# rezashkv/unlearn-ft

Measured on AMD Instinct MI355X. Metric: bilevel train-step images/sec @512^2 pruned-SD2.1, higher is better.
Workload: dtype bf16; 1 GPU; BASELINE configs[1] model+batch (MAC-budget-0.55 SD-2.1 student [ratio 0.556, 223.7 GMAC/img] + dense teacher [402.1 GMAC/img], B=8/GPU, 64x64 latents = 512^2 px, losses 1.0 ddpm(min-SNR 5) + 2.0 distill + 0.1 block) under the bilevel cadence of configs[2] (upper concept-suppression step every 10th iteration, second AdamW); global_batch=8, parallelism=dp1, student_params=483766084, weights=random-init, attention_precision=activation dtype, dist_backend=none, rccl_ranks=0, dp_mode=allreduce, teacher_prefetch=True

## Files before the change

unlearn-ft_amd/csrc/attention.hip:

```cpp
#include <cstdlib>

#include "common.h"

namespace {

constexpr int NT = 256;
constexpr int D = 64;
constexpr float LOG2E = 1.4426950408889634f;
typedef __attribute__((ext_vector_type(4))) unsigned u32x4;
typedef __attribute__((ext_vector_type(2))) float f32x2;
constexpr unsigned OOB = 0x80000000u;

#ifndef PDMK_ATTN_KVB
#define PDMK_ATTN_KVB 64
#endif
template <typename T> struct ACfg;
template <> struct ACfg<bf16> {
    static constexpr int CH = 8, RS = 64, KVB = PDMK_ATTN_KVB;
};
template <> struct ACfg<float> {
    static constexpr int CH = 4, RS = 68, KVB = 32;
};

template <typename T> struct AT;
template <> struct AT<bf16> {
    typedef Mma<bf16> MM;
    static constexpr int RS = 64;
    static __device__ __forceinline__ int sw(int row) { return row & 7; }
    static __device__ __forceinline__ MM::frag rowk(const bf16* lds, int row0, int k0, int lane) {
        const int row = row0 + (lane & 15), ch = ((k0 >> 3) + (lane >> 4)) ^ (row & 7);
        return *reinterpret_cast<const bf16x8*>(lds + row * RS + ch * 8);
    }
    template <int S> static __device__ __forceinline__ MM::frag colk_accs(const bf16* lds, int k0, int col0, int lane) {
        const int g = lane >> 4, q = (lane & 15) >> 2, p = lane & 3;
        const int row = k0 + 4 * g + q;
        const bf16* a0 = lds + row * RS + ((((col0 >> 3) + (p >> 1)) ^ (row & 7)) * 8) + (p & 1) * 4;
        typedef __attribute__((address_space(3))) s16x4 lds_s16x4;
        s16x4 lo = __builtin_amdgcn_ds_read_tr16_b64_v4i16((lds_s16x4*)(a0));
        s16x4 hi = __builtin_amdgcn_ds_read_tr16_b64_v4i16((lds_s16x4*)(a0 + 16 * RS));
        s16x8 v = __builtin_shufflevector(lo, hi, 0, 1, 2, 3, 4, 5, 6, 7);
        return __builtin_bit_cast(bf16x8, v);
    }
};
template <> struct AT<float> {
    typedef Mma<float> MM;
    static constexpr int RS = 68;
    static __device__ __forceinline__ int sw(int) { return 0; }
    static __device__ __forceinline__ MM::frag rowk(const float* lds, int row0, int k0, int lane) {
        return MM::load_rowk(lds, RS, row0, k0, lane);
    }
    template <int S> static __device__ __forceinline__ MM::frag colk_accs(const float* lds, int k0, int col0, int lane) {
        return MM::template load_colk_accs<S>(lds, RS, k0, col0, lane);
    }
};

template <typename T, int ROWS> struct TileIO {
    static constexpr int CH = ACfg<T>::CH, RS = ACfg<T>::RS, CPR = D / CH, NR = ROWS * CPR / NT;
    static_assert(ROWS * CPR % NT == 0, "tile chunks must divide the block");
    template <typename RS_T>
    static __device__ __forceinline__ void load(u32x4* r, const RS_T& rsrc, int ld, int row0, int nrows, int tid) {
#pragma unroll
        for (int i = 0; i < NR; ++i) {
            const int c = tid + i * NT, row = row0 + c / CPR, dc = (c % CPR) * CH;
            const unsigned off = row < nrows ? ((unsigned)row * (unsigned)ld + (unsigned)dc) * (unsigned)sizeof(T) : OOB;
            r[i] = __builtin_amdgcn_raw_buffer_load_b128(rsrc, (int)off, 0, 0);
        }
    }
    static __device__ __forceinline__ void store(T* lds, const u32x4* r, int tid) {
#pragma unroll
        for (int i = 0; i < NR; ++i) {
            const int c = tid + i * NT, row = c / CPR;
            *reinterpret_cast<u32x4*>(lds + row * RS + (((c % CPR) ^ AT<T>::sw(row)) * CH)) = r[i];
        }
    }
};

template <typename T> __device__ __forceinline__ auto make_rsrc(const T* p, long nrows, int ld) {
    const long bytes = ((nrows - 1) * (long)ld + D) * (long)sizeof(T);
    return __builtin_amdgcn_make_buffer_rsrc(const_cast<T*>(p), (short)0, (int)bytes, 0x00020000);
}

template <typename T>
__device__ __forceinline__ void store_tile16(const T* lds, T* g, long ld, int row0, int nrows, int lane) {
    constexpr int CH = ACfg<T>::CH, RS = ACfg<T>::RS, CPR = D / CH;
    for (int c = lane; c < 16 * CPR; c += 64) {
        const int r = c / CPR, dc = (c % CPR) * CH;
        if (row0 + r < nrows)
            *reinterpret_cast<uint4*>(g + (long)(row0 + r) * ld + dc) = *reinterpret_cast<const uint4*>(lds + r * RS + dc);
    }
}
template <typename T>
__device__ __forceinline__ void stage_t(T* lds, const f32x4* acc, float scale, int lane) {
    constexpr int RS = ACfg<T>::RS;
#pragma unroll
    for (int dt = 0; dt < 4; ++dt)
#pragma unroll
        for (int r = 0; r < 4; ++r)
            lds[(lane & 15) * RS + dt * 16 + (lane >> 4) * 4 + r] = from_f32<T>(acc[dt][r] * scale);
}

template <typename MM, int S, int NS> struct AccLoop {
    template <typename F> static __device__ __forceinline__ void run(F&& f) {
        f(std::integral_constant<int, S>{});
        AccLoop<MM, S + 1, NS>::run(f);
    }
};
template <typename MM, int NS> struct AccLoop<MM, NS, NS> {
    template <typename F> static __device__ __forceinline__ void run(F&&) {}
};

template <typename T> struct BlockSums : std::is_same<T, float> {};

template <typename T, int NQ, bool CAUSAL = false>
__global__ __launch_bounds__(NT) void attn_fwd_kernel(const T* __restrict__ q, const T* __restrict__ k,
                                                      const T* __restrict__ v, T* __restrict__ o,
                                                      float* __restrict__ lse, int H, int Nq, int Nk, long q_bs,
                                                      int q_ld, long k_bs, int k_ld, long v_bs, int v_ld, long o_bs,
                                                      int o_ld, float scale2) {
    typedef Mma<T> MM;
    typedef ACfg<T> AC;
    constexpr int RS = AC::RS, KVB = AC::KVB, NKT = KVB / 16, QROWS = 64 * NQ;
    constexpr bool BLOCK_SUMS = BlockSums<T>::value;
    typedef TileIO<T, QROWS> QIO;
    typedef TileIO<T, KVB> KIO;
    __shared__ __attribute__((aligned(16))) T Qs[QROWS * RS];
    __shared__ __attribute__((aligned(16))) T Ks[2][KVB * RS];
    __shared__ __attribute__((aligned(16))) T Vs[2][KVB * RS];

    const int tid = threadIdx.x, lane = tid & 63, wave = tid >> 6;
    const int q0 = blockIdx.x * QROWS, h = blockIdx.y, b = blockIdx.z;
    const auto rq = make_rsrc(q + b * q_bs + h * D, Nq, q_ld);
    const auto rk = make_rsrc(k + b * k_bs + h * D, Nk, k_ld);
    const auto rv = make_rsrc(v + b * v_bs + h * D, Nk, v_ld);

    u32x4 rk_[KIO::NR], rv_[KIO::NR];
    {
        u32x4 rq_[QIO::NR];
        QIO::load(rq_, rq, q_ld, q0, Nq, tid);
        KIO::load(rk_, rk, k_ld, 0, Nk, tid);
        KIO::load(rv_, rv, v_ld, 0, Nk, tid);
        QIO::store(Qs, rq_, tid);
    }
    KIO::store(Ks[0], rk_, tid);
    KIO::store(Vs[0], rv_, tid);
    __syncthreads();
    typename MM::frag qf[NQ][D / MM::KS];
#pragma unroll
    for (int n = 0; n < NQ; ++n)
#pragma unroll
        for (int kk = 0; kk < D / MM::KS; ++kk) qf[n][kk] = AT<T>::rowk(Qs, (wave * NQ + n) * 16, kk * MM::KS, lane);

    f32x4 ot[NQ][4], ol[NQ];
    float m_run[NQ];
#pragma unroll
    for (int n = 0; n < NQ; ++n) {
        m_run[n] = -INFINITY;
        ol[n] = f32x4{0.f, 0.f, 0.f, 0.f};
#pragma unroll
        for (int i = 0; i < 4; ++i) ot[n][i] = f32x4{0.f, 0.f, 0.f, 0.f};
    }
    typename MM::frag ones;
    if constexpr (std::is_same<T, bf16>::value) {
#pragma unroll
        for (int e = 0; e < 8; ++e) ones[e] = (bf16)1.0f;
    } else {
        ones = 1.0f;
    }

    int cur = 0;
    auto block = [&](auto tail_c, const int kb) {
        constexpr bool TAIL = decltype(tail_c)::value;
        const bool more = kb + KVB < Nk;
        if (more) {
            KIO::load(rk_, rk, k_ld, kb + KVB, Nk, tid);
            KIO::load(rv_, rv, v_ld, kb + KVB, Nk, tid);
        }
        f32x4 st[NQ][NKT];
#pragma unroll
        for (int t = 0; t < NKT; ++t) {
#pragma unroll
            for (int n = 0; n < NQ; ++n) st[n][t] = f32x4{0.f, 0.f, 0.f, 0.f};
#pragma unroll
            for (int kk = 0; kk < D / MM::KS; ++kk) {
                const typename MM::frag kf = AT<T>::rowk(Ks[cur], t * 16, kk * MM::KS, lane);
#pragma unroll
                for (int n = 0; n < NQ; ++n) st[n][t] = MM::mma(kf, qf[n][kk], st[n][t]);
            }
        }
#pragma unroll
        for (int n = 0; n < NQ; ++n) {
            float mx = -INFINITY;
            if (TAIL) {
#pragma unroll
                for (int t = 0; t < NKT; ++t)
#pragma unroll
                    for (int r = 0; r < 4; ++r)
                        if (kb + t * 16 + (lane >> 4) * 4 + r >= Nk) st[n][t][r] = -INFINITY;
            }
            if (CAUSAL) {
                const int qi = q0 + (wave * NQ + n) * 16 + (lane & 15);
#pragma unroll
                for (int t = 0; t < NKT; ++t)
#pragma unroll
                    for (int r = 0; r < 4; ++r)
                        if (kb + t * 16 + (lane >> 4) * 4 + r > qi) st[n][t][r] = -INFINITY;
            }
#pragma unroll
            for (int t = 0; t < NKT; ++t)
#pragma unroll
                for (int r = 0; r < 4; ++r) mx = fmaxf(mx, st[n][t][r]);
            mx = fmaxf(mx, __shfl_xor(mx, 16, 64));
            mx = fmaxf(mx, __shfl_xor(mx, 32, 64));
            const float mxs = mx * scale2;
            const bool move = mxs > m_run[n] + 8.0f;
            if (__builtin_amdgcn_ballot_w64(move)) {
                const float mn = move ? mxs : m_run[n];
                const float alpha = __builtin_amdgcn_exp2f(m_run[n] - mn);
                m_run[n] = mn;
#pragma unroll
                for (int r = 0; r < 4; ++r) ol[n][r] *= alpha;
#pragma unroll
                for (int dt = 0; dt < 4; ++dt)
#pragma unroll
                    for (int r = 0; r < 4; ++r) ot[n][dt][r] *= alpha;
            }
            const f32x2 sc2 = {scale2, scale2}, nm2 = {-m_run[n], -m_run[n]};
#pragma unroll
            for (int t = 0; t < NKT; ++t)
#pragma unroll
                for (int r = 0; r < 4; r += 2) {
                    const f32x2 e2 = __builtin_elementwise_fma(f32x2{st[n][t][r], st[n][t][r + 1]}, sc2, nm2);
                    st[n][t][r] = __builtin_amdgcn_exp2f(e2[0]);
                    st[n][t][r + 1] = __builtin_amdgcn_exp2f(e2[1]);
                }
        }
        f32x4 otb[BLOCK_SUMS ? NQ : 1][4], olb[BLOCK_SUMS ? NQ : 1];
        if constexpr (BLOCK_SUMS) {
#pragma unroll
            for (int n = 0; n < NQ; ++n) {
                olb[n] = f32x4{0.f, 0.f, 0.f, 0.f};
#pragma unroll
                for (int i = 0; i < 4; ++i) otb[n][i] = f32x4{0.f, 0.f, 0.f, 0.f};
            }
        }
#pragma unroll
        for (int pr = 0; pr < NKT / 2; ++pr) {
            AccLoop<MM, 0, MM::ACC_STEPS>::run([&](auto sc) {
                constexpr int S = decltype(sc)::value;
                typename MM::frag pf[NQ];
#pragma unroll
                for (int n = 0; n < NQ; ++n) {
                    pf[n] = MM::template acc_frag<S>(st[n][2 * pr], st[n][2 * pr + 1]);
                    if constexpr (BLOCK_SUMS) olb[n] = MM::mma(ones, pf[n], olb[n]);
                    else ol[n] = MM::mma(ones, pf[n], ol[n]);
                }
#pragma unroll
                for (int dt = 0; dt < 4; ++dt) {
                    const typename MM::frag vf = AT<T>::template colk_accs<S>(Vs[cur], pr * 32, dt * 16, lane);
#pragma unroll
                    for (int n = 0; n < NQ; ++n) {
                        if constexpr (BLOCK_SUMS) otb[n][dt] = MM::mma(vf, pf[n], otb[n][dt]);
                        else ot[n][dt] = MM::mma(vf, pf[n], ot[n][dt]);
                    }
                }
            });
        }
        if constexpr (BLOCK_SUMS) {
#pragma unroll
            for (int n = 0; n < NQ; ++n) {
                ol[n] += olb[n];
#pragma unroll
                for (int dt = 0; dt < 4; ++dt) ot[n][dt] += otb[n][dt];
            }
        }
        if (more) {
            KIO::store(Ks[cur ^ 1], rk_, tid);
            KIO::store(Vs[cur ^ 1], rv_, tid);
        }
        __syncthreads();
        cur ^= 1;
    };
    const int nfull = Nk / KVB * KVB;
    for (int kb = 0; kb < nfull; kb += KVB) block(std::false_type{}, kb);
    if (nfull < Nk) block(std::true_type{}, nfull);
#pragma unroll
    for (int n = 0; n < NQ; ++n) {
        const float l = ol[n][0];
        T* Ow = Qs + (wave * NQ + n) * 16 * RS;
        stage_t<T>(Ow, ot[n], 1.0f / l, lane);
        const int qi = q0 + (wave * NQ + n) * 16 + (lane & 15);
        if (lane < 16 && qi < Nq) lse[((long)b * H + h) * Nq + qi] = m_run[n] + log2f(l);
    }
    __syncthreads();
#pragma unroll
    for (int n = 0; n < NQ; ++n)
        store_tile16<T>(Qs + (wave * NQ + n) * 16 * RS, o + b * o_bs + h * D, o_ld, q0 + (wave * NQ + n) * 16, Nq, lane);
}

template <typename T>
__global__ void attn_delta_kernel(const T* __restrict__ o, const T* __restrict__ d_o, float* __restrict__ delta, int H,
                                  int Nq, long o_bs, int o_ld, long total) {
    constexpr int CH = ACfg<T>::CH;
    for (long i = blockIdx.x * (long)NT + threadIdx.x; i < total; i += (long)gridDim.x * NT) {
        const int qi = (int)(i % Nq);
        const long bh = i / Nq;
        const int h = (int)(bh % H);
        const long b = bh / H;
        const T* po = o + b * o_bs + (long)qi * o_ld + h * D;
        const T* pd = d_o + b * o_bs + (long)qi * o_ld + h * D;
        float s = 0.f;
#pragma unroll
        for (int c = 0; c < D; c += CH) {
            const uint4 a = *reinterpret_cast<const uint4*>(po + c), g = *reinterpret_cast<const uint4*>(pd + c);
            const T* ae = reinterpret_cast<const T*>(&a);
            const T* ge = reinterpret_cast<const T*>(&g);
#pragma unroll
            for (int e = 0; e < CH; ++e) s += to_f32(ae[e]) * to_f32(ge[e]);
        }
        delta[i] = s;
    }
}

template <typename T, bool SPLIT, int NKW>
__global__ __launch_bounds__(NT) void attn_bwd_dkv_kernel(const T* __restrict__ q, const T* __restrict__ k,
                                                          const T* __restrict__ v, const T* __restrict__ d_o,
                                                          const float* __restrict__ lse,
                                                          const float* __restrict__ delta, T* __restrict__ dk,
                                                          T* __restrict__ dv, int H, int Nq, int Nk, long q_bs,
                                                          int q_ld, long k_bs, int k_ld, long v_bs, int v_ld,
                                                          long o_bs, int o_ld, long dk_bs, int dk_ld, long dv_bs,
                                                          int dv_ld, float scale, float scale2, float* __restrict__ ws,
                                                          int nsplit) {
    typedef Mma<T> MM;
    typedef ACfg<T> AC;
    constexpr int RS = AC::RS, QB = AC::KVB, NQT = QB / 16, KROWS = 64 * NKW;
    constexpr bool BLOCK_SUMS = BlockSums<T>::value;
    typedef TileIO<T, KROWS> KIO;
    typedef TileIO<T, QB> QIO;
    static_assert(!SPLIT || NKW == 1, "the query split is for few-key grids");
    __shared__ __attribute__((aligned(16))) T Ks[KROWS * RS];
    __shared__ __attribute__((aligned(16))) T Vs[KROWS * RS];
    __shared__ __attribute__((aligned(16))) T Qs[2][QB * RS];
    __shared__ __attribute__((aligned(16))) T Os[2][QB * RS];
    __shared__ __attribute__((aligned(16))) float Ls[2][QB], Ds[2][QB];

    const int tid = threadIdx.x, lane = tid & 63, wave = tid >> 6;
    const int kblocks = (Nk + KROWS - 1) / KROWS;
    const int split = SPLIT ? blockIdx.x / kblocks : 0;
    const int k0 = (SPLIT ? blockIdx.x - split * kblocks : blockIdx.x) * KROWS, h = blockIdx.y, b = blockIdx.z;
    int q_begin = 0, q_end = Nq;
    if (SPLIT) {
        const int nqb = (Nq + QB - 1) / QB, per = (nqb + nsplit - 1) / nsplit;
        q_begin = min(Nq, split * per * QB);
        q_end = min(Nq, (split + 1) * per * QB);
    }
    const auto rq = make_rsrc(q + b * q_bs + h * D, Nq, q_ld);
    const auto ro = make_rsrc(d_o + b * o_bs + h * D, Nq, o_ld);
    const auto rk = make_rsrc(k + b * k_bs + h * D, Nk, k_ld);
    const auto rv = make_rsrc(v + b * v_bs + h * D, Nk, v_ld);
    const float* lse_bh = lse + ((long)b * H + h) * Nq;
    const float* del_bh = delta + ((long)b * H + h) * Nq;

    u32x4 rq_[QIO::NR], ro_[QIO::NR];
    float rl = -INFINITY, rd = 0.f;
    {
        u32x4 rk_[KIO::NR], rv_[KIO::NR];
        KIO::load(rk_, rk, k_ld, k0, Nk, tid);
        KIO::load(rv_, rv, v_ld, k0, Nk, tid);
        QIO::load(rq_, rq, q_ld, q_begin, Nq, tid);
        QIO::load(ro_, ro, o_ld, q_begin, Nq, tid);
        if (tid < QB && q_begin + tid < Nq) { rl = -lse_bh[q_begin + tid]; rd = -del_bh[q_begin + tid]; }
        KIO::store(Ks, rk_, tid);
        KIO::store(Vs, rv_, tid);
    }
    QIO::store(Qs[0], rq_, tid);
    QIO::store(Os[0], ro_, tid);
    if (tid < QB) { Ls[0][tid] = rl; Ds[0][tid] = rd; }
    __syncthreads();
    typename MM::frag kf[NKW][D / MM::KS], vf[NKW][D / MM::KS];
    f32x4 dkt[NKW][4], dvt[NKW][4];
#pragma unroll
    for (int j = 0; j < NKW; ++j) {
#pragma unroll
        for (int kk = 0; kk < D / MM::KS; ++kk) {
            kf[j][kk] = AT<T>::rowk(Ks, (wave * NKW + j) * 16, kk * MM::KS, lane);
            vf[j][kk] = AT<T>::rowk(Vs, (wave * NKW + j) * 16, kk * MM::KS, lane);
        }
#pragma unroll
        for (int i = 0; i < 4; ++i) { dkt[j][i] = f32x4{0.f, 0.f, 0.f, 0.f}; dvt[j][i] = f32x4{0.f, 0.f, 0.f, 0.f}; }
    }

    int cur = 0;
    for (int qb = q_begin; qb < q_end; qb += QB) {
        const bool more = qb + QB < q_end;
        if (more) {
            QIO::load(rq_, rq, q_ld, qb + QB, Nq, tid);
            QIO::load(ro_, ro, o_ld, qb + QB, Nq, tid);
            rl = -INFINITY; rd = 0.f;
            if (tid < QB && qb + QB + tid < Nq) { rl = -lse_bh[qb + QB + tid]; rd = -del_bh[qb + QB + tid]; }
        }
        f32x4 p[NKW][NQT], ds[NKW][NQT];
#pragma unroll
        for (int t = 0; t < NQT; ++t) {
            f32x4 sacc[NKW], dp[NKW];
            const f32x4 nd = *reinterpret_cast<const f32x4*>(&Ds[cur][t * 16 + (lane >> 4) * 4]);
            const f32x4 nlv = *reinterpret_cast<const f32x4*>(&Ls[cur][t * 16 + (lane >> 4) * 4]);
#pragma unroll
            for (int j = 0; j < NKW; ++j) { sacc[j] = f32x4{0.f, 0.f, 0.f, 0.f}; dp[j] = BLOCK_SUMS ? f32x4{0.f, 0.f, 0.f, 0.f} : nd; }
#pragma unroll
            for (int kk = 0; kk < D / MM::KS; ++kk) {
                const typename MM::frag qa = AT<T>::rowk(Qs[cur], t * 16, kk * MM::KS, lane);
                const typename MM::frag oa = AT<T>::rowk(Os[cur], t * 16, kk * MM::KS, lane);
#pragma unroll
                for (int j = 0; j < NKW; ++j) {
                    sacc[j] = MM::mma(qa, kf[j][kk], sacc[j]);
                    dp[j] = MM::mma(oa, vf[j][kk], dp[j]);
                }
            }
#pragma unroll
            for (int r = 0; r < 4; r += 2) {
#pragma unroll
                for (int j = 0; j < NKW; ++j) {
                    const f32x2 e2 = __builtin_elementwise_fma(f32x2{sacc[j][r], sacc[j][r + 1]}, f32x2{scale2, scale2}, f32x2{nlv[r], nlv[r + 1]});
                    const f32x2 pv = {__builtin_amdgcn_exp2f(e2[0]), __builtin_amdgcn_exp2f(e2[1])};
                    f32x2 dpd = {dp[j][r], dp[j][r + 1]};
                    if constexpr (BLOCK_SUMS) dpd += f32x2{nd[r], nd[r + 1]};
                    const f32x2 d2 = pv * dpd;
                    p[j][t][r] = pv[0];
                    p[j][t][r + 1] = pv[1];
                    ds[j][t][r] = d2[0];
                    ds[j][t][r + 1] = d2[1];
                }
            }
        }
        f32x4 dkb[BLOCK_SUMS ? NKW : 1][4], dvb[BLOCK_SUMS ? NKW : 1][4];
        if constexpr (BLOCK_SUMS) {
#pragma unroll
            for (int j = 0; j < NKW; ++j)
#pragma unroll
                for (int i = 0; i < 4; ++i) { dkb[j][i] = f32x4{0.f, 0.f, 0.f, 0.f}; dvb[j][i] = f32x4{0.f, 0.f, 0.f, 0.f}; }
        }
#pragma unroll
        for (int pr = 0; pr < NQT / 2; ++pr) {
            AccLoop<MM, 0, MM::ACC_STEPS>::run([&](auto sc) {
                constexpr int S = decltype(sc)::value;
                typename MM::frag pf[NKW], sf[NKW];
#pragma unroll
                for (int j = 0; j < NKW; ++j) {
                    pf[j] = MM::template acc_frag<S>(p[j][2 * pr], p[j][2 * pr + 1]);
                    sf[j] = MM::template acc_frag<S>(ds[j][2 * pr], ds[j][2 * pr + 1]);
                }
#pragma unroll
                for (int dt = 0; dt < 4; ++dt) {
                    const typename MM::frag oc = AT<T>::template colk_accs<S>(Os[cur], pr * 32, dt * 16, lane);
                    const typename MM::frag qc = AT<T>::template colk_accs<S>(Qs[cur], pr * 32, dt * 16, lane);
#pragma unroll
                    for (int j = 0; j < NKW; ++j) {
                        if constexpr (BLOCK_SUMS) {
                            dvb[j][dt] = MM::mma(oc, pf[j], dvb[j][dt]);
                            dkb[j][dt] = MM::mma(qc, sf[j], dkb[j][dt]);
                        } else {
                            dvt[j][dt] = MM::mma(oc, pf[j], dvt[j][dt]);
                            dkt[j][dt] = MM::mma(qc, sf[j], dkt[j][dt]);
                        }
                    }
                }
            });
        }
        if constexpr (BLOCK_SUMS) {
#pragma unroll
            for (int j = 0; j < NKW; ++j)
#pragma unroll
                for (int dt = 0; dt < 4; ++dt) { dvt[j][dt] += dvb[j][dt]; dkt[j][dt] += dkb[j][dt]; }
        }
        if (more) {
            QIO::store(Qs[cur ^ 1], rq_, tid);
            QIO::store(Os[cur ^ 1], ro_, tid);
            if (tid < QB) { Ls[cur ^ 1][tid] = rl; Ds[cur ^ 1][tid] = rd; }
        }
        __syncthreads();
        cur ^= 1;
    }
    if (SPLIT) {
        const int key = k0 + wave * 16 + (lane & 15);
        if (key < Nk) {
            const long slab = ((((long)split * 2) * gridDim.z + b) * H + h) * Nk + key;
            const long dv_off = (long)gridDim.z * H * Nk;
#pragma unroll
            for (int dt = 0; dt < 4; ++dt) {
                f32x4 a = dkt[0][dt];
#pragma unroll
                for (int r = 0; r < 4; ++r) a[r] *= scale;
                *reinterpret_cast<f32x4*>(ws + slab * 64 + dt * 16 + (lane >> 4) * 4) = a;
                *reinterpret_cast<f32x4*>(ws + (slab + dv_off) * 64 + dt * 16 + (lane >> 4) * 4) = dvt[0][dt];
            }
        }
        return;
    }
#pragma unroll
    for (int j = 0; j < NKW; ++j) {
        stage_t<T>(Ks + (wave * NKW + j) * 16 * RS, dkt[j], scale, lane);
        stage_t<T>(Vs + (wave * NKW + j) * 16 * RS, dvt[j], 1.0f, lane);
    }
    __syncthreads();
#pragma unroll
    for (int j = 0; j < NKW; ++j) {
        store_tile16<T>(Ks + (wave * NKW + j) * 16 * RS, dk + b * dk_bs + h * D, dk_ld, k0 + (wave * NKW + j) * 16, Nk, lane);
        store_tile16<T>(Vs + (wave * NKW + j) * 16 * RS, dv + b * dv_bs + h * D, dv_ld, k0 + (wave * NKW + j) * 16, Nk, lane);
    }
}

template <typename T, int NQ>
__global__ __launch_bounds__(NT) void attn_bwd_dq_kernel(const T* __restrict__ q, const T* __restrict__ k,
                                                         const T* __restrict__ v, const T* __restrict__ o,
                                                         const T* __restrict__ d_o,
                                                         const float* __restrict__ lse,
                                                         float* __restrict__ delta, T* __restrict__ dq, int H,
                                                         int Nq, int Nk, long q_bs, int q_ld, long k_bs, int k_ld,
                                                         long v_bs, int v_ld, long o_bs, int o_ld, long dq_bs,
                                                         int dq_ld, float scale, float scale2) {
    typedef Mma<T> MM;
    typedef ACfg<T> AC;
    constexpr int RS = AC::RS, KVB = AC::KVB, NKT = KVB / 16, QROWS = 64 * NQ;
    constexpr bool BLOCK_SUMS = BlockSums<T>::value;
    constexpr bool DELTA_SWEEP = std::is_same<T, float>::value;
    typedef TileIO<T, QROWS> QIO;
    typedef TileIO<T, KVB> KIO;
    __shared__ __attribute__((aligned(16))) T Qs[QROWS * RS];
    __shared__ __attribute__((aligned(16))) T Os[QROWS * RS];
    __shared__ __attribute__((aligned(16))) T Ks[2][KVB * RS];
    __shared__ __attribute__((aligned(16))) T Vs[2][KVB * RS];
    __shared__ float dls[QROWS];

    const int tid = threadIdx.x, lane = tid & 63, wave = tid >> 6;
    const int q0 = blockIdx.x * QROWS, h = blockIdx.y, b = blockIdx.z;
    const auto rq = make_rsrc(q + b * q_bs + h * D, Nq, q_ld);
    const auto ro = make_rsrc(d_o + b * o_bs + h * D, Nq, o_ld);
    const auto rO = make_rsrc(o + b * o_bs + h * D, Nq, o_ld);
    const auto rk = make_rsrc(k + b * k_bs + h * D, Nk, k_ld);
    const auto rv = make_rsrc(v + b * v_bs + h * D, Nk, v_ld);

    u32x4 rk_[KIO::NR], rv_[KIO::NR];
    {
        u32x4 rq_[QIO::NR], ro_[QIO::NR], rO_[QIO::NR];
        QIO::load(rq_, rq, q_ld, q0, Nq, tid);
        QIO::load(ro_, ro, o_ld, q0, Nq, tid);
        QIO::load(rO_, rO, o_ld, q0, Nq, tid);
        KIO::load(rk_, rk, k_ld, 0, Nk, tid);
        KIO::load(rv_, rv, v_ld, 0, Nk, tid);
        QIO::store(Qs, rq_, tid);
        QIO::store(Os, ro_, tid);
        constexpr int CPR = QIO::CPR, CH = QIO::CH;
#pragma unroll
        for (int i = 0; i < QIO::NR; ++i) {
            const T* a = reinterpret_cast<const T*>(&ro_[i]);
            const T* c_ = reinterpret_cast<const T*>(&rO_[i]);
            float s_ = 0.f;
#pragma unroll
            for (int e = 0; e < CH; ++e) s_ += to_f32(a[e]) * to_f32(c_[e]);
#pragma unroll
            for (int m = 1; m < CPR; m <<= 1) s_ += __shfl_xor(s_, m, 64);
            const int c = tid + i * NT, row = c / CPR;
            if ((c % CPR) == 0) {
                dls[row] = s_;
                if (!DELTA_SWEEP && q0 + row < Nq) delta[((long)b * H + h) * Nq + q0 + row] = s_;
            }
        }
    }
    KIO::store(Ks[0], rk_, tid);
    KIO::store(Vs[0], rv_, tid);
    __syncthreads();
    typename MM::frag qf[NQ][D / MM::KS], of[NQ][D / MM::KS];
    float nl2[NQ], ndl[NQ];
    f32x4 dqt[NQ][4];
#pragma unroll
    for (int n = 0; n < NQ; ++n) {
#pragma unroll
        for (int kk = 0; kk < D / MM::KS; ++kk) {
            qf[n][kk] = AT<T>::rowk(Qs, (wave * NQ + n) * 16, kk * MM::KS, lane);
            of[n][kk] = AT<T>::rowk(Os, (wave * NQ + n) * 16, kk * MM::KS, lane);
        }
        const int qi = q0 + (wave * NQ + n) * 16 + (lane & 15);
        nl2[n] = qi < Nq ? -lse[((long)b * H + h) * Nq + qi] : -INFINITY;
        ndl[n] = qi < Nq ? -dls[(wave * NQ + n) * 16 + (lane & 15)] : 0.f;
#pragma unroll
        for (int i = 0; i < 4; ++i) dqt[n][i] = f32x4{0.f, 0.f, 0.f, 0.f};
    }

    int cur = 0;
    double dacc[NQ], zacc[NQ];
#pragma unroll
    for (int n = 0; n < NQ; ++n) dacc[n] = zacc[n] = 0.f;
    auto block = [&](auto tail_c, auto first_c, const int kb) {
        constexpr bool TAIL = decltype(tail_c)::value, FIRST = decltype(first_c)::value;
        const bool more = FIRST || kb + KVB < Nk;
        const int nxt = FIRST && kb + KVB >= Nk ? 0 : kb + KVB;
        if (more) {
            KIO::load(rk_, rk, k_ld, nxt, Nk, tid);
            KIO::load(rv_, rv, v_ld, nxt, Nk, tid);
        }
        f32x4 dst[NQ][NKT];
#pragma unroll
        for (int t = 0; t < NKT; ++t) {
            f32x4 s[NQ], dp[NQ];
#pragma unroll
            for (int n = 0; n < NQ; ++n) {
                s[n] = f32x4{0.f, 0.f, 0.f, 0.f};
                const float d0 = (FIRST || DELTA_SWEEP) ? 0.f : ndl[n];
                dp[n] = f32x4{d0, d0, d0, d0};
            }
#pragma unroll
            for (int kk = 0; kk < D / MM::KS; ++kk) {
                const typename MM::frag kf = AT<T>::rowk(Ks[cur], t * 16, kk * MM::KS, lane);
                const typename MM::frag vf = AT<T>::rowk(Vs[cur], t * 16, kk * MM::KS, lane);
#pragma unroll
                for (int n = 0; n < NQ; ++n) {
                    s[n] = MM::mma(kf, qf[n][kk], s[n]);
                    dp[n] = MM::mma(vf, of[n][kk], dp[n]);
                }
            }
#pragma unroll
            for (int n = 0; n < NQ; ++n)
#pragma unroll
                for (int r = 0; r < 4; r += 2) {
                    const f32x2 e2 = __builtin_elementwise_fma(f32x2{s[n][r], s[n][r + 1]}, f32x2{scale2, scale2}, f32x2{nl2[n], nl2[n]});
                    f32x2 pv = {__builtin_amdgcn_exp2f(e2[0]), __builtin_amdgcn_exp2f(e2[1])};
                    if (TAIL) {
                        if (kb + t * 16 + (lane >> 4) * 4 + r >= Nk) pv[0] = 0.f;
                        if (kb + t * 16 + (lane >> 4) * 4 + r + 1 >= Nk) pv[1] = 0.f;
                    }
                    f32x2 dpd = {dp[n][r], dp[n][r + 1]};
                    if constexpr (DELTA_SWEEP && !FIRST) dpd += f32x2{ndl[n], ndl[n]};
                    const f32x2 d2 = pv * dpd;
                    if constexpr (FIRST) {
                        dacc[n] += (double)pv[0] * (double)dp[n][r] + (double)pv[1] * (double)dp[n][r + 1];
                        zacc[n] += (double)pv[0] + (double)pv[1];
                    } else {
                        dst[n][t][r] = d2[0];
                        dst[n][t][r + 1] = d2[1];
                    }
                }
        }
        if constexpr (!FIRST) {
        f32x4 dqb[BLOCK_SUMS ? NQ : 1][4];
        if constexpr (BLOCK_SUMS) {
#pragma unroll
            for (int n = 0; n < NQ; ++n)
#pragma unroll
                for (int i = 0; i < 4; ++i) dqb[n][i] = f32x4{0.f, 0.f, 0.f, 0.f};
        }
#pragma unroll
        for (int pr = 0; pr < NKT / 2; ++pr) {
            AccLoop<MM, 0, MM::ACC_STEPS>::run([&](auto sc) {
                constexpr int S = decltype(sc)::value;
                typename MM::frag sf[NQ];
#pragma unroll
                for (int n = 0; n < NQ; ++n) sf[n] = MM::template acc_frag<S>(dst[n][2 * pr], dst[n][2 * pr + 1]);
#pragma unroll
                for (int dt = 0; dt < 4; ++dt) {
                    const typename MM::frag kc = AT<T>::template colk_accs<S>(Ks[cur], pr * 32, dt * 16, lane);
#pragma unroll
                    for (int n = 0; n < NQ; ++n) {
                        if constexpr (BLOCK_SUMS) dqb[n][dt] = MM::mma(kc, sf[n], dqb[n][dt]);
                        else dqt[n][dt] = MM::mma(kc, sf[n], dqt[n][dt]);
                    }
                }
            });
        }
        if constexpr (BLOCK_SUMS) {
#pragma unroll
            for (int n = 0; n < NQ; ++n)
#pragma unroll
                for (int dt = 0; dt < 4; ++dt) dqt[n][dt] += dqb[n][dt];
        }
        }
        if (more) {
            KIO::store(Ks[cur ^ 1], rk_, tid);
            KIO::store(Vs[cur ^ 1], rv_, tid);
        }
        __syncthreads();
        cur ^= 1;
    };
    const int nfull = Nk / KVB * KVB;
    if constexpr (DELTA_SWEEP) {
        for (int kb = 0; kb < nfull; kb += KVB) block(std::false_type{}, std::true_type{}, kb);
        if (nfull < Nk) block(std::true_type{}, std::true_type{}, nfull);
#pragma unroll
        for (int n = 0; n < NQ; ++n) {
            double dd = dacc[n], z = zacc[n];
            dd += __shfl_xor(dd, 16, 64);
            z += __shfl_xor(z, 16, 64);
            dd += __shfl_xor(dd, 32, 64);
            z += __shfl_xor(z, 32, 64);
            const int qi = q0 + (wave * NQ + n) * 16 + (lane & 15);
            const float d = qi < Nq ? (float)(dd / z) : 0.f;
            ndl[n] = -d;
            if (lane < 16 && qi < Nq) delta[((long)b * H + h) * Nq + qi] = d;
        }
    }
    for (int kb = 0; kb < nfull; kb += KVB) block(std::false_type{}, std::false_type{}, kb);
    if (nfull < Nk) block(std::true_type{}, std::false_type{}, nfull);
#pragma unroll
    for (int n = 0; n < NQ; ++n) stage_t<T>(Qs + (wave * NQ + n) * 16 * RS, dqt[n], scale, lane);
    __syncthreads();
#pragma unroll
    for (int n = 0; n < NQ; ++n)
        store_tile16<T>(Qs + (wave * NQ + n) * 16 * RS, dq + b * dq_bs + h * D, dq_ld, q0 + (wave * NQ + n) * 16, Nq, lane);
}

template <typename T>
__global__ void attn_dkv_reduce_kernel(const float* __restrict__ ws, T* __restrict__ dk, T* __restrict__ dv, int B, int H,
                                       int Nk, int nsplit, long dk_bs, int dk_ld, long dv_bs, int dv_ld) {
    const long total = (long)2 * B * H * Nk * 16;
    const long i = (long)blockIdx.x * NT + threadIdx.x;
    if (i >= total) return;
    float4 a = *reinterpret_cast<const float4*>(ws + i * 4);
    for (int s = 1; s < nsplit; ++s) {
        const float4 u = *reinterpret_cast<const float4*>(ws + ((long)s * total + i) * 4);
        a.x += u.x; a.y += u.y; a.z += u.z; a.w += u.w;
    }
    const int d4 = (int)(i & 15);
    long r = i >> 4;
    const int key = (int)(r % Nk); r /= Nk;
    const int h = (int)(r % H); r /= H;
    const int b = (int)(r % B);
    const bool is_v = r / B != 0;
    T* o = (is_v ? dv + b * dv_bs + (long)key * dv_ld : dk + b * dk_bs + (long)key * dk_ld) + h * D + d4 * 4;
    o[0] = from_f32<T>(a.x); o[1] = from_f32<T>(a.y); o[2] = from_f32<T>(a.z); o[3] = from_f32<T>(a.w);
}

thread_local int g_fwd_form = 0, g_dq_form = 0, g_dkv_form = 0, g_nsplit = 0;

template <typename T> bool aligned_ok(const void* p, long bs, int ld, long nrows) {
    constexpr int CH = ACfg<T>::CH;
    return (((uintptr_t)p) & 15) == 0 && (bs % CH) == 0 && (ld % CH) == 0 &&
           ((nrows - 1) * (long)ld + D) * (long)sizeof(T) < (1L << 31);
}

template <typename T>
int attn_fwd(const void* q, const void* k, const void* v, void* o, float* lse, int B, int H, int Nq, int Nk, long q_bs,
             int q_ld, long k_bs, int k_ld, long v_bs, int v_ld, long o_bs, int o_ld, float scale, int causal, hipStream_t st) {
    if (!aligned_ok<T>(q, q_bs, q_ld, Nq) || !aligned_ok<T>(k, k_bs, k_ld, Nk) || !aligned_ok<T>(v, v_bs, v_ld, Nk) ||
        !aligned_ok<T>(o, o_bs, o_ld, Nq))
        return -1;
    if (causal) {
        hipLaunchKernelGGL((attn_fwd_kernel<T, 1, true>), dim3((Nq + 63) / 64, H, B), dim3(NT), 0, st, (const T*)q, (const T*)k,
                           (const T*)v, (T*)o, lse, H, Nq, Nk, q_bs, q_ld, k_bs, k_ld, v_bs, v_ld, o_bs, o_ld, scale * LOG2E);
        PDMK_CHECK_LAUNCH();
        g_fwd_form = 1;
        return 0;
    }
    static int forced = -1, dynamic = -1;
    if (dynamic < 0) dynamic = getenv("PDMK_ENV_DYNAMIC") ? 1 : 0;
    if (forced < 0 || dynamic) { const char* e = getenv("PDMK_ATTN_NQ"); forced = e ? atoi(e) : 0; }
    const bool wide = forced ? forced == 2 : ((long)((Nq + 127) / 128) * H * B >= 384 && Nk >= 256);
    if (wide) {
        hipLaunchKernelGGL((attn_fwd_kernel<T, 2>), dim3((Nq + 127) / 128, H, B), dim3(NT), 0, st, (const T*)q, (const T*)k,
                           (const T*)v, (T*)o, lse, H, Nq, Nk, q_bs, q_ld, k_bs, k_ld, v_bs, v_ld, o_bs, o_ld, scale * LOG2E);
    } else {
        hipLaunchKernelGGL((attn_fwd_kernel<T, 1>), dim3((Nq + 63) / 64, H, B), dim3(NT), 0, st, (const T*)q, (const T*)k,
                           (const T*)v, (T*)o, lse, H, Nq, Nk, q_bs, q_ld, k_bs, k_ld, v_bs, v_ld, o_bs, o_ld, scale * LOG2E);
    }
    PDMK_CHECK_LAUNCH();
    g_fwd_form = wide ? 2 : 1;
    return 0;
}

template <typename T>
int attn_bwd(const void* q, const void* k, const void* v, const void* o, const void* d_o, const float* lse,
             float* delta, void* dq, void* dk, void* dv, int B, int H, int Nq, int Nk, long q_bs, int q_ld, long k_bs,
             int k_ld, long v_bs, int v_ld, long o_bs, int o_ld, long dq_bs, int dq_ld, long dk_bs, int dk_ld,
             long dv_bs, int dv_ld, float scale, float* ws, long ws_elems, hipStream_t st) {
    if (!aligned_ok<T>(q, q_bs, q_ld, Nq) || !aligned_ok<T>(k, k_bs, k_ld, Nk) || !aligned_ok<T>(v, v_bs, v_ld, Nk) ||
        !aligned_ok<T>(o, o_bs, o_ld, Nq) || !aligned_ok<T>(d_o, o_bs, o_ld, Nq) || !aligned_ok<T>(dq, dq_bs, dq_ld, Nq) ||
        !aligned_ok<T>(dk, dk_bs, dk_ld, Nk) || !aligned_ok<T>(dv, dv_bs, dv_ld, Nk))
        return -1;
    static int forced = -1, dynamic = -1;
    if (dynamic < 0) dynamic = getenv("PDMK_ENV_DYNAMIC") ? 1 : 0;
    if (forced < 0 || dynamic) { const char* e = getenv("PDMK_ATTN_NQ"); forced = e ? atoi(e) : 0; }
#define PDMK_DQ_ARGS (const T*)q, (const T*)k, (const T*)v, (const T*)o, (const T*)d_o, lse, delta, (T*)dq, H, Nq, Nk, q_bs, q_ld, k_bs, k_ld, \
                     v_bs, v_ld, o_bs, o_ld, dq_bs, dq_ld, scale, scale * LOG2E
    static int f_dq = -1, f_dkv = -1;
    if (f_dq < 0 || dynamic) {
        const char* e = getenv("PDMK_ATTN_NQ_DQ");
        f_dq = e ? atoi(e) : 0;
        e = getenv("PDMK_ATTN_NQ_DKV");
        f_dkv = e ? atoi(e) : 0;
    }
    constexpr bool is_bf16 = std::is_same<T, bf16>::value;
    const int want_dq = f_dq ? f_dq : forced, want_dkv = f_dkv ? f_dkv : forced;
#ifdef PDMK_ATTN_AGPR
    const bool auto_wide = false;
#else
    const bool auto_wide = true;
#endif
    const bool wide_dq = is_bf16 && (want_dq ? want_dq == 2 : (auto_wide && (long)((Nq + 127) / 128) * H * B >= 384 && Nk >= 256));
    const bool wide_dkv = is_bf16 && (want_dkv ? want_dkv == 2 : (auto_wide && (long)((Nk + 127) / 128) * H * B >= 384 && Nq >= 256));
    constexpr int BW = is_bf16 ? 2 : 1;
    if (wide_dq)
        hipLaunchKernelGGL((attn_bwd_dq_kernel<T, BW>), dim3((Nq + 127) / 128, H, B), dim3(NT), 0, st, PDMK_DQ_ARGS);
    else
        hipLaunchKernelGGL((attn_bwd_dq_kernel<T, 1>), dim3((Nq + 63) / 64, H, B), dim3(NT), 0, st, PDMK_DQ_ARGS);
#undef PDMK_DQ_ARGS
    const int kblocks = (Nk + 63) / 64, qblocks = (Nq + ACfg<T>::KVB - 1) / ACfg<T>::KVB;
    int nsplit = 1;
    if (ws && kblocks * H * B < 128 && qblocks >= 8) {
        nsplit = min(min(32, qblocks / 4), (256 + kblocks * H * B - 1) / (kblocks * H * B));
        const long per = (long)2 * B * H * Nk * 64;
        if (nsplit > ws_elems / per) nsplit = max(1, (int)(ws_elems / per));
    }
#define PDMK_DKV_ARGS (const T*)q, (const T*)k, (const T*)v, (const T*)d_o, lse, delta, (T*)dk, (T*)dv, H, Nq, Nk, q_bs, q_ld, \
                      k_bs, k_ld, v_bs, v_ld, o_bs, o_ld, dk_bs, dk_ld, dv_bs, dv_ld, scale, scale * LOG2E
    if (nsplit > 1) {
        hipLaunchKernelGGL((attn_bwd_dkv_kernel<T, true, 1>), dim3(kblocks * nsplit, H, B), dim3(NT), 0, st, PDMK_DKV_ARGS, ws,
                           nsplit);
        const long items = (long)2 * B * H * Nk * 16;
        hipLaunchKernelGGL(attn_dkv_reduce_kernel<T>, dim3((unsigned)((items + NT - 1) / NT)), dim3(NT), 0, st, ws, (T*)dk,
                           (T*)dv, B, H, Nk, nsplit, dk_bs, dk_ld, dv_bs, dv_ld);
    } else if (wide_dkv) {
        hipLaunchKernelGGL((attn_bwd_dkv_kernel<T, false, BW>), dim3((Nk + 127) / 128, H, B), dim3(NT), 0, st, PDMK_DKV_ARGS,
                           nullptr, 1);
    } else {
        hipLaunchKernelGGL((attn_bwd_dkv_kernel<T, false, 1>), dim3(kblocks, H, B), dim3(NT), 0, st, PDMK_DKV_ARGS, nullptr, 1);
    }
#undef PDMK_DKV_ARGS
    PDMK_CHECK_LAUNCH();
    g_dq_form = wide_dq ? 2 : 1;
    g_dkv_form = nsplit > 1 ? 1 : (wide_dkv ? 2 : 1);
    g_nsplit = nsplit;
    return 0;
}

}

extern "C" int pdmk_attn_fwd(const void* q, const void* k, const void* v, void* o, float* lse, int B, int H, int Nq,
                             int Nk, int64_t q_bs, int q_ld, int64_t k_bs, int k_ld, int64_t v_bs, int v_ld,
                             int64_t o_bs, int o_ld, float scale, int dtype, pdmk_stream stream) {
    if (!q || !k || !v || !o || !lse || B <= 0 || H <= 0 || Nq <= 0 || Nk <= 0) return -1;
    hipStream_t st = (hipStream_t)stream;
    if (dtype == PDMK_BF16)
        return attn_fwd<bf16>(q, k, v, o, lse, B, H, Nq, Nk, q_bs, q_ld, k_bs, k_ld, v_bs, v_ld, o_bs, o_ld, scale, 0, st);
    if (dtype == PDMK_F32)
        return attn_fwd<float>(q, k, v, o, lse, B, H, Nq, Nk, q_bs, q_ld, k_bs, k_ld, v_bs, v_ld, o_bs, o_ld, scale, 0, st);
    return -2;
}

extern "C" int pdmk_attn_fwd_causal(const void* q, const void* k, const void* v, void* o, float* lse, int B, int H, int N,
                                    int64_t q_bs, int q_ld, int64_t k_bs, int k_ld, int64_t v_bs, int v_ld, int64_t o_bs,
                                    int o_ld, float scale, int dtype, pdmk_stream stream) {
    if (!q || !k || !v || !o || !lse || B <= 0 || H <= 0 || N <= 0) return -1;
    hipStream_t st = (hipStream_t)stream;
    if (dtype == PDMK_BF16)
        return attn_fwd<bf16>(q, k, v, o, lse, B, H, N, N, q_bs, q_ld, k_bs, k_ld, v_bs, v_ld, o_bs, o_ld, scale, 1, st);
    if (dtype == PDMK_F32)
        return attn_fwd<float>(q, k, v, o, lse, B, H, N, N, q_bs, q_ld, k_bs, k_ld, v_bs, v_ld, o_bs, o_ld, scale, 1, st);
    return -2;
}

extern "C" int pdmk_attn_bwd(const void* q, const void* k, const void* v, const void* o, const void* d_o,
                             const float* lse, float* delta, void* dq, void* dk, void* dv, int B, int H, int Nq,
                             int Nk, int64_t q_bs, int q_ld, int64_t k_bs, int k_ld, int64_t v_bs, int v_ld,
                             int64_t o_bs, int o_ld, int64_t dq_bs, int dq_ld, int64_t dk_bs, int dk_ld,
                             int64_t dv_bs, int dv_ld, float scale, float* ws, int64_t ws_elems, int dtype,
                             pdmk_stream stream) {
    if (!q || !k || !v || !o || !d_o || !lse || !delta || !dq || !dk || !dv || B <= 0 || H <= 0 || Nq <= 0 || Nk <= 0)
        return -1;
    hipStream_t st = (hipStream_t)stream;
    if (dtype == PDMK_BF16)
        return attn_bwd<bf16>(q, k, v, o, d_o, lse, delta, dq, dk, dv, B, H, Nq, Nk, q_bs, q_ld, k_bs, k_ld, v_bs, v_ld,
                              o_bs, o_ld, dq_bs, dq_ld, dk_bs, dk_ld, dv_bs, dv_ld, scale, ws, (long)ws_elems, st);
    if (dtype == PDMK_F32)
        return attn_bwd<float>(q, k, v, o, d_o, lse, delta, dq, dk, dv, B, H, Nq, Nk, q_bs, q_ld, k_bs, k_ld, v_bs,
                               v_ld, o_bs, o_ld, dq_bs, dq_ld, dk_bs, dk_ld, dv_bs, dv_ld, scale, ws, (long)ws_elems, st);
    return -2;
}

extern "C" int pdmk_attn_last_forms(void) {
    return g_fwd_form | (g_dq_form << 4) | (g_dkv_form << 8) | (g_nsplit << 12);
}
```

Measured before the change: 191.4 images/s.

## Add short-key attention kernels that keep all K/V in LDS and sweep query blocks

```diff
diff --git a/unlearn-ft_amd/csrc/attention.hip b/unlearn-ft_amd/csrc/attention.hip
--- a/unlearn-ft_amd/csrc/attention.hip
+++ b/unlearn-ft_amd/csrc/attention.hip
@@ -708,6 +708,295 @@
         store_tile16<T>(Qs + (wave * NQ + n) * 16 * RS, dq + b * dq_bs + h * D, dq_ld, q0 + (wave * NQ + n) * 16, Nq, lane);
 }
 
+constexpr int SK_MAX = 128;
+
+__device__ __forceinline__ void wave_sync() {
+    __builtin_amdgcn_fence(__ATOMIC_ACQ_REL, "wavefront");
+    __builtin_amdgcn_wave_barrier();
+}
+
+template <typename T> struct WaveTile {
+    static constexpr int CH = ACfg<T>::CH, RS = ACfg<T>::RS, CPR = D / CH, NR = 16 * CPR / 64;
+    template <typename RS_T>
+    static __device__ __forceinline__ void load(u32x4* r, const RS_T& rsrc, int ld, int row0, int nrows, int lane) {
+#pragma unroll
+        for (int i = 0; i < NR; ++i) {
+            const int c = lane + i * 64, row = row0 + c / CPR, dc = (c % CPR) * CH;
+            const unsigned off = row < nrows ? ((unsigned)row * (unsigned)ld + (unsigned)dc) * (unsigned)sizeof(T) : OOB;
+            r[i] = __builtin_amdgcn_raw_buffer_load_b128(rsrc, (int)off, 0, 0);
+        }
+    }
+    static __device__ __forceinline__ void store(T* lds, const u32x4* r, int lane) {
+#pragma unroll
+        for (int i = 0; i < NR; ++i) {
+            const int c = lane + i * 64, row = c / CPR;
+            *reinterpret_cast<u32x4*>(lds + row * RS + (((c % CPR) ^ AT<T>::sw(row)) * CH)) = r[i];
+        }
+    }
+};
+
+template <typename T, int ROWS, typename RS_T>
+__device__ __forceinline__ void load_key_images(T* Ks, T* Vs, const RS_T& rk, int k_ld, const RS_T& rv, int v_ld, int Nk, int tid) {
+    typedef TileIO<T, ROWS> KIO;
+    u32x4 rk_[KIO::NR], rv_[KIO::NR];
+    KIO::load(rk_, rk, k_ld, 0, Nk, tid);
+    KIO::load(rv_, rv, v_ld, 0, Nk, tid);
+    KIO::store(Ks, rk_, tid);
+    KIO::store(Vs, rv_, tid);
+}
+
+template <typename T, int NTL>
+__global__ __launch_bounds__(NT) void attn_fwd_short_kernel(const T* __restrict__ q, const T* __restrict__ k,
+                                                            const T* __restrict__ v, T* __restrict__ o,
+                                                            float* __restrict__ lse, int H, int Nq, int Nk, long q_bs,
+                                                            int q_ld, long k_bs, int k_ld, long v_bs, int v_ld, long o_bs,
+                                                            int o_ld, float scale2, int sweep) {
+    typedef Mma<T> MM;
+    typedef WaveTile<T> WIO;
+    constexpr int RS = ACfg<T>::RS, NPL = (NTL + 1) / 2, NKT = 2 * NPL, KROWS = 16 * NKT;
+    __shared__ __attribute__((aligned(16))) T Ks[KROWS * RS];
+    __shared__ __attribute__((aligned(16))) T Vs[KROWS * RS];
+    __shared__ __attribute__((aligned(16))) T Qs[64 * RS];
+
+    const int tid = threadIdx.x, lane = tid & 63, wave = tid >> 6;
+    const int h = blockIdx.y, b = blockIdx.z;
+    const int nqb = (Nq + 63) / 64, blk0 = blockIdx.x * sweep, blk1 = min(nqb, blk0 + sweep);
+    const auto rq = make_rsrc(q + b * q_bs + h * D, Nq, q_ld);
+    const auto rk = make_rsrc(k + b * k_bs + h * D, Nk, k_ld);
+    const auto rv = make_rsrc(v + b * v_bs + h * D, Nk, v_ld);
+    T* Qw = Qs + wave * 16 * RS;
+
+    u32x4 rq_[WIO::NR];
+    WIO::load(rq_, rq, q_ld, blk0 * 64 + wave * 16, Nq, lane);
+    load_key_images<T, KROWS>(Ks, Vs, rk, k_ld, rv, v_ld, Nk, tid);
+    WIO::store(Qw, rq_, lane);
+    __syncthreads();
+    typename MM::frag ones;
+    if constexpr (std::is_same<T, bf16>::value) {
+#pragma unroll
+        for (int e = 0; e < 8; ++e) ones[e] = (bf16)1.0f;
+    } else {
+        ones = 1.0f;
+    }
+
+    for (int blk = blk0; blk < blk1; ++blk) {
+        const int q0 = blk * 64 + wave * 16;
+        const bool more = blk + 1 < blk1;
+        typename MM::frag qf[D / MM::KS];
+#pragma unroll
+        for (int kk = 0; kk < D / MM::KS; ++kk) qf[kk] = AT<T>::rowk(Qw, 0, kk * MM::KS, lane);
+        if (more) WIO::load(rq_, rq, q_ld, q0 + 64, Nq, lane);
+        f32x4 st[NKT];
+        float mx = -INFINITY;
+#pragma unroll
+        for (int t = 0; t < NTL; ++t) {
+            f32x4 acc = {0.f, 0.f, 0.f, 0.f};
+#pragma unroll
+            for (int kk = 0; kk < D / MM::KS; ++kk)
+                acc = MM::mma(AT<T>::rowk(Ks, t * 16, kk * MM::KS, lane), qf[kk], acc);
+            if (t == NTL - 1) {
+#pragma unroll
+                for (int r = 0; r < 4; ++r) acc[r] = t * 16 + (lane >> 4) * 4 + r >= Nk ? -INFINITY : acc[r];
+            }
+#pragma unroll
+            for (int r = 0; r < 4; ++r) mx = fmaxf(mx, acc[r]);
+            st[t] = acc;
+        }
+        if (NTL < NKT) st[NKT - 1] = f32x4{0.f, 0.f, 0.f, 0.f};
+        mx = fmaxf(mx, __shfl_xor(mx, 16, 64));
+        mx = fmaxf(mx, __shfl_xor(mx, 32, 64));
+        const float m = mx * scale2;
+        const f32x2 sc2 = {scale2, scale2}, nm2 = {-m, -m};
+        f32x4 ot[4], ol = {0.f, 0.f, 0.f, 0.f};
+#pragma unroll
+        for (int i = 0; i < 4; ++i) ot[i] = f32x4{0.f, 0.f, 0.f, 0.f};
+#pragma unroll
+        for (int t = 0; t < NTL; ++t)
+#pragma unroll
+            for (int r = 0; r < 4; r += 2) {
+                const f32x2 e2 = __builtin_elementwise_fma(f32x2{st[t][r], st[t][r + 1]}, sc2, nm2);
+                st[t][r] = __builtin_amdgcn_exp2f(e2[0]);
+                st[t][r + 1] = __builtin_amdgcn_exp2f(e2[1]);
+            }
+#pragma unroll
+        for (int pr = 0; pr < NPL; ++pr) {
+            AccLoop<MM, 0, MM::ACC_STEPS>::run([&](auto sc) {
+                constexpr int S = decltype(sc)::value;
+                const typename MM::frag pf = MM::template acc_frag<S>(st[2 * pr], st[2 * pr + 1]);
+                ol = MM::mma(ones, pf, ol);
+#pragma unroll
+                for (int dt = 0; dt < 4; ++dt)
+                    ot[dt] = MM::mma(AT<T>::template colk_accs<S>(Vs, pr * 32, dt * 16, lane), pf, ot[dt]);
+            });
+        }
+        const float l = ol[0];
+        wave_sync();
+        stage_t<T>(Qw, ot, 1.0f / l, lane);
+        const int qi = q0 + (lane & 15);
+        if (lane < 16 && qi < Nq) lse[((long)b * H + h) * Nq + qi] = m + log2f(l);
+        wave_sync();
+        store_tile16<T>(Qw, o + b * o_bs + h * D, o_ld, q0, Nq, lane);
+        wave_sync();
+        if (more) WIO::store(Qw, rq_, lane);
+        wave_sync();
+    }
+}
+
+template <typename T, int NTL>
+__global__ __launch_bounds__(NT) void attn_bwd_dq_short_kernel(const T* __restrict__ q, const T* __restrict__ k,
+                                                               const T* __restrict__ v, const T* __restrict__ o,
+                                                               const T* __restrict__ d_o,
+                                                               const float* __restrict__ lse,
+                                                               float* __restrict__ delta, T* __restrict__ dq, int H,
+                                                               int Nq, int Nk, long q_bs, int q_ld, long k_bs, int k_ld,
+                                                               long v_bs, int v_ld, long o_bs, int o_ld, long dq_bs,
+                                                               int dq_ld, float scale, float scale2, int sweep) {
+    typedef Mma<T> MM;
+    typedef WaveTile<T> WIO;
+    constexpr int RS = ACfg<T>::RS, NPL = (NTL + 1) / 2, NKT = 2 * NPL, KROWS = 16 * NKT;
+    constexpr bool F32 = std::is_same<T, float>::value;
+    __shared__ __attribute__((aligned(16))) T Ks[KROWS * RS];
+    __shared__ __attribute__((aligned(16))) T Vs[KROWS * RS];
+    __shared__ __attribute__((aligned(16))) T Qs[64 * RS];
+    __shared__ __attribute__((aligned(16))) T Os[64 * RS];
+
+    const int tid = threadIdx.x, lane = tid & 63, wave = tid >> 6;
+    const int h = blockIdx.y, b = blockIdx.z;
+    const int nqb = (Nq + 63) / 64, blk0 = blockIdx.x * sweep, blk1 = min(nqb, blk0 + sweep);
+    const auto rq = make_rsrc(q + b * q_bs + h * D, Nq, q_ld);
+    const auto ro = make_rsrc(d_o + b * o_bs + h * D, Nq, o_ld);
+    const auto rO = make_rsrc(o + b * o_bs + h * D, Nq, o_ld);
+    const auto rk = make_rsrc(k + b * k_bs + h * D, Nk, k_ld);
+    const auto rv = make_rsrc(v + b * v_bs + h * D, Nk, v_ld);
+    const float* lse_bh = lse + ((long)b * H + h) * Nq;
+    float* del_bh = delta + ((long)b * H + h) * Nq;
+    T* Qw = Qs + wave * 16 * RS;
+    T* Ow = Os + wave * 16 * RS;
+
+    u32x4 rq_[WIO::NR], ro_[WIO::NR], rO_[F32 ? 1 : WIO::NR];
+    float rl = -INFINITY;
+    auto fetch = [&](const int q0) {
+        WIO::load(rq_, rq, q_ld, q0, Nq, lane);
+        WIO::load(ro_, ro, o_ld, q0, Nq, lane);
+        if constexpr (!F32) WIO::load(rO_, rO, o_ld, q0, Nq, lane);
+        const int qi = q0 + (lane & 15);
+        rl = qi < Nq ? -lse_bh[qi] : -INFINITY;
+    };
+    float nl2 = -INFINITY, ndl = 0.f;
+    auto publish = [&](const int q0) {
+        WIO::store(Qw, rq_, lane);
+        WIO::store(Ow, ro_, lane);
+        nl2 = rl;
+        if constexpr (!F32) {
+            constexpr int CPR = WIO::CPR, CH = WIO::CH, RPI = 64 / CPR;
+            static_assert(WIO::NR == 2 && RPI == 8, "row r of the tile: part[r / 8] of lane (r % 8) * CPR");
+            float part[WIO::NR];
+#pragma unroll
+            for (int i = 0; i < WIO::NR; ++i) {
+                const T* a = reinterpret_cast<const T*>(&ro_[i]);
+                const T* c_ = reinterpret_cast<const T*>(&rO_[i]);
+                float s_ = 0.f;
+#pragma unroll
+                for (int e = 0; e < CH; ++e) s_ += to_f32(a[e]) * to_f32(c_[e]);
+#pragma unroll
+                for (int m_ = 1; m_ < CPR; m_ <<= 1) s_ += __shfl_xor(s_, m_, 64);
+                const int row = (lane + i * 64) / CPR;
+                if ((lane % CPR) == 0 && q0 + row < Nq) del_bh[q0 + row] = s_;
+                part[i] = s_;
+            }
+            const float d0 = __shfl(part[0], (lane & 7) * CPR, 64), d1 = __shfl(part[1], (lane & 7) * CPR, 64);
+            ndl = q0 + (lane & 15) < Nq ? -((lane & 8) ? d1 : d0) : 0.f;
+        }
+    };
+
+    fetch(blk0 * 64 + wave * 16);
+    load_key_images<T, KROWS>(Ks, Vs, rk, k_ld, rv, v_ld, Nk, tid);
+    publish(blk0 * 64 + wave * 16);
+    __syncthreads();
+
+    for (int blk = blk0; blk < blk1; ++blk) {
+        const int q0 = blk * 64 + wave * 16;
+        const bool more = blk + 1 < blk1;
+        typename MM::frag qf[D / MM::KS], of[D / MM::KS];
+#pragma unroll
+        for (int kk = 0; kk < D / MM::KS; ++kk) {
+            qf[kk] = AT<T>::rowk(Qw, 0, kk * MM::KS, lane);
+            of[kk] = AT<T>::rowk(Ow, 0, kk * MM::KS, lane);
+        }
+        if (more) fetch(q0 + 64);
+        f32x4 dst[NKT], dps[F32 ? NKT : 1];
+        double dacc = 0.0, zacc = 0.0;
+#pragma unroll
+        for (int t = 0; t < NTL; ++t) {
+            const float d0 = F32 ? 0.f : ndl;
+            f32x4 s = {0.f, 0.f, 0.f, 0.f}, dp = {d0, d0, d0, d0};
+#pragma unroll
+            for (int kk = 0; kk < D / MM::KS; ++kk) {
+                s = MM::mma(AT<T>::rowk(Ks, t * 16, kk * MM::KS, lane), qf[kk], s);
+                dp = MM::mma(AT<T>::rowk(Vs, t * 16, kk * MM::KS, lane), of[kk], dp);
+            }
+#pragma unroll
+            for (int r = 0; r < 4; r += 2) {
+                const f32x2 e2 = __builtin_elementwise_fma(f32x2{s[r], s[r + 1]}, f32x2{scale2, scale2}, f32x2{nl2, nl2});
+                f32x2 pv = {__builtin_amdgcn_exp2f(e2[0]), __builtin_amdgcn_exp2f(e2[1])};
+                if (t == NTL - 1) {
+                    pv[0] = t * 16 + (lane >> 4) * 4 + r >= Nk ? 0.f : pv[0];
+                    pv[1] = t * 16 + (lane >> 4) * 4 + r + 1 >= Nk ? 0.f : pv[1];
+                }
+                if constexpr (F32) {
+                    dacc += (double)pv[0] * (double)dp[r] + (double)pv[1] * (double)dp[r + 1];
+                    zacc += (double)pv[0] + (double)pv[1];
+                    dst[t][r] = pv[0];
+                    dst[t][r + 1] = pv[1];
+                } else {
+                    const f32x2 d2 = pv * f32x2{dp[r], dp[r + 1]};
+                    dst[t][r] = d2[0];
+                    dst[t][r + 1] = d2[1];
+                }
+            }
+            if constexpr (F32) dps[t] = dp;
+        }
+        if (NTL < NKT) dst[NKT - 1] = f32x4{0.f, 0.f, 0.f, 0.f};
+        if constexpr (F32) {
+            dacc += __shfl_xor(dacc, 16, 64);
+            zacc += __shfl_xor(zacc, 16, 64);
+            dacc += __shfl_xor(dacc, 32, 64);
+            zacc += __shfl_xor(zacc, 32, 64);
+            const int qi = q0 + (lane & 15);
+            const float d = qi < Nq ? (float)(dacc / zacc) : 0.f;
+            if (lane < 16 && qi < Nq) del_bh[qi] = d;
+#pragma unroll
+            for (int t = 0; t < NTL; ++t)
+#pragma unroll
+                for (int r = 0; r < 4; r += 2) {
+                    const f32x2 d2 = f32x2{dst[t][r], dst[t][r + 1]} * (f32x2{dps[t][r], dps[t][r + 1]} + f32x2{-d, -d});
+                    dst[t][r] = d2[0];
+                    dst[t][r + 1] = d2[1];
+                }
+        }
+        f32x4 dqt[4];
+#pragma unroll
+        for (int i = 0; i < 4; ++i) dqt[i] = f32x4{0.f, 0.f, 0.f, 0.f};
+#pragma unroll
+        for (int pr = 0; pr < NPL; ++pr) {
+            AccLoop<MM, 0, MM::ACC_STEPS>::run([&](auto sc) {
+                constexpr int S = decltype(sc)::value;
+                const typename MM::frag sf = MM::template acc_frag<S>(dst[2 * pr], dst[2 * pr + 1]);
+#pragma unroll
+                for (int dt = 0; dt < 4; ++dt)
+                    dqt[dt] = MM::mma(AT<T>::template colk_accs<S>(Ks, pr * 32, dt * 16, lane), sf, dqt[dt]);
+            });
+        }
+        wave_sync();
+        stage_t<T>(Qw, dqt, scale, lane);
+        wave_sync();
+        store_tile16<T>(Qw, dq + b * dq_bs + h * D, dq_ld, q0, Nq, lane);
+        wave_sync();
+        if (more) publish(q0 + 64);
+        wave_sync();
+    }
+}
+
 template <typename T>
 __global__ void attn_dkv_reduce_kernel(const float* __restrict__ ws, T* __restrict__ dk, T* __restrict__ dv, int B, int H,
                                        int Nk, int nsplit, long dk_bs, int dk_ld, long dv_bs, int dv_ld) {
@@ -730,6 +1019,28 @@
 }
 
 thread_local int g_fwd_form = 0, g_dq_form = 0, g_dkv_form = 0, g_nsplit = 0;
+
+int attn_qsweep(int nqb, int H, int B, int wg_per_cu) {
+    static int forced = -1, dynamic = -1;
+    if (dynamic < 0) dynamic = getenv("PDMK_ENV_DYNAMIC") ? 1 : 0;
+    if (forced < 0 || dynamic) { const char* e = getenv("PDMK_ATTN_QSWEEP"); forced = e ? atoi(e) : 0; }
+    const long s = forced > 0 ? forced : (long)nqb * H * B / (2L * 256 * wg_per_cu);
+    return (int)max(1L, min(s, (long)nqb));
+}
+template <typename T> int short_wg_per_cu(int tiles, int ntl) {
+    return (int)min(4L, 160L * 1024 / ((2L * 32 * ((ntl + 1) / 2) + 64L * tiles) * ACfg<T>::RS * (long)sizeof(T)));
+}
+#define PDMK_SHORT_LAUNCH(kern, ntl, grid, ...)                                                                              \
+    switch (ntl) {                                                                                                           \
+        case 1: hipLaunchKernelGGL((kern<T, 1>), grid, dim3(NT), 0, st, __VA_ARGS__); break;                                 \
+        case 2: hipLaunchKernelGGL((kern<T, 2>), grid, dim3(NT), 0, st, __VA_ARGS__); break;                                 \
+        case 3: hipLaunchKernelGGL((kern<T, 3>), grid, dim3(NT), 0, st, __VA_ARGS__); break;                                 \
+        case 4: hipLaunchKernelGGL((kern<T, 4>), grid, dim3(NT), 0, st, __VA_ARGS__); break;                                 \
+        case 5: hipLaunchKernelGGL((kern<T, 5>), grid, dim3(NT), 0, st, __VA_ARGS__); break;                                 \
+        case 6: hipLaunchKernelGGL((kern<T, 6>), grid, dim3(NT), 0, st, __VA_ARGS__); break;                                 \
+        case 7: hipLaunchKernelGGL((kern<T, 7>), grid, dim3(NT), 0, st, __VA_ARGS__); break;                                 \
+        default: hipLaunchKernelGGL((kern<T, 8>), grid, dim3(NT), 0, st, __VA_ARGS__); break;                                \
+    }
 
 template <typename T> bool aligned_ok(const void* p, long bs, int ld, long nrows) {
     constexpr int CH = ACfg<T>::CH;
@@ -754,7 +1065,11 @@
     if (dynamic < 0) dynamic = getenv("PDMK_ENV_DYNAMIC") ? 1 : 0;
     if (forced < 0 || dynamic) { const char* e = getenv("PDMK_ATTN_NQ"); forced = e ? atoi(e) : 0; }
     const bool wide = forced ? forced == 2 : ((long)((Nq + 127) / 128) * H * B >= 384 && Nk >= 256);
-    if (wide) {
+    if (!wide && Nk <= SK_MAX) {
+        const int ntl = (Nk + 15) / 16, nqb = (Nq + 63) / 64, sweep = attn_qsweep(nqb, H, B, short_wg_per_cu<T>(1, ntl));
+        PDMK_SHORT_LAUNCH(attn_fwd_short_kernel, ntl, dim3((nqb + sweep - 1) / sweep, H, B), (const T*)q, (const T*)k,
+                          (const T*)v, (T*)o, lse, H, Nq, Nk, q_bs, q_ld, k_bs, k_ld, v_bs, v_ld, o_bs, o_ld, scale * LOG2E, sweep);
+    } else if (wide) {
         hipLaunchKernelGGL((attn_fwd_kernel<T, 2>), dim3((Nq + 127) / 128, H, B), dim3(NT), 0, st, (const T*)q, (const T*)k,
                            (const T*)v, (T*)o, lse, H, Nq, Nk, q_bs, q_ld, k_bs, k_ld, v_bs, v_ld, o_bs, o_ld, scale * LOG2E);
     } else {
@@ -797,7 +1112,10 @@
     const bool wide_dq = is_bf16 && (want_dq ? want_dq == 2 : (auto_wide && (long)((Nq + 127) / 128) * H * B >= 384 && Nk >= 256));
     const bool wide_dkv = is_bf16 && (want_dkv ? want_dkv == 2 : (auto_wide && (long)((Nk + 127) / 128) * H * B >= 384 && Nq >= 256));
     constexpr int BW = is_bf16 ? 2 : 1;
-    if (wide_dq)
+    if (!wide_dq && Nk <= SK_MAX) {
+        const int ntl = (Nk + 15) / 16, nqb = (Nq + 63) / 64, sweep = attn_qsweep(nqb, H, B, short_wg_per_cu<T>(2, ntl));
+        PDMK_SHORT_LAUNCH(attn_bwd_dq_short_kernel, ntl, dim3((nqb + sweep - 1) / sweep, H, B), PDMK_DQ_ARGS, sweep);
+    } else if (wide_dq)
         hipLaunchKernelGGL((attn_bwd_dq_kernel<T, BW>), dim3((Nq + 127) / 128, H, B), dim3(NT), 0, st, PDMK_DQ_ARGS);
     else
         hipLaunchKernelGGL((attn_bwd_dq_kernel<T, 1>), dim3((Nq + 63) / 64, H, B), dim3(NT), 0, st, PDMK_DQ_ARGS);
```

Result: no change. 191.8 images/s (median of 3 runs) (+0.2%).
